# libsdl-org/libjxl

Hardware: AMD Instinct MI355X
Metric: megapixels/sec decode, 3840x2160 VarDCT d1.0 (higher is better)
Workload: dtype f32

## Files before the change

### libjxl_amd/csrc/hip/jxl_hip_entropy_lanes.h

```cpp
#ifndef JXL_HIP_ENTROPY_LANES_H_
#define JXL_HIP_ENTROPY_LANES_H_

#include "jxl_hip_kernels.h"
#include "jxl_hip_lanes_trip.inc"

namespace jxlhip {

struct EntropyLaneBatch {
  const EntropyParams* params;
  const uint32_t* wg_unit;
  const uint4* units;
  const uint32_t* list;
  uint32_t* queue;
  const uint8_t* wave_lanes;
  uint32_t prio;
  uint32_t extra_pass_min;
  uint32_t wait_shift;
  uint32_t refill_mask;
  const uint8_t* wave_log_ls;
  uint32_t debug;
  unsigned long long* started;
  unsigned long long* prof;
};

struct LanesLds {
  uint32_t f2, alias, ctx, ctx2, cfg, poff, wave0, per_wave, total;
};
constexpr uint32_t kLanesF2Bytes = 128;
constexpr uint32_t kLanesNzRows = 96;
constexpr uint32_t kLanesRingWords = 16;
constexpr uint32_t kLanesBlockRing = 8;
constexpr int kLanesTrips = 4;
constexpr uint32_t kLanesRefillEvery = 4;
constexpr uint32_t kLanesPerLaneBytes = kLanesNzRows + (kLanesRingWords + 2) * 4 + kLanesBlockRing * 4;
constexpr uint32_t kLanesA6Clusters = 128, kLanesA6Slots = 8192, kLanesA6B = 128, kLanesA6A = kLanesA6B + kLanesA6Slots * 2,
                   kLanesA6Cfg = kLanesA6A + kLanesA6Slots * 4, kLanesA6End = kLanesA6Cfg + kLanesA6Clusters * 2;
static_assert(kLanesA6A == 16512 && kLanesA6Cfg == 49280, "jxl_hip_lanes_trip.inc LT_EREAD_6 has these as immediates");
__host__ __device__ inline LanesLds LanesLdsLayout(uint32_t num_hist, uint32_t nctx, uint32_t num_clusters, uint32_t log_alpha,
                                                   uint32_t waves, uint32_t lanes, bool alias_lds = true, bool prefix = false, bool a6 = false) {
  LanesLds l;
  l.f2 = 0;
  l.alias = kLanesF2Bytes;
  l.ctx = a6 ? kLanesA6End : l.alias + (alias_lds ? (num_clusters << log_alpha) * 8 : 0);
  l.ctx2 = l.ctx + ((num_hist * nctx + 16 + 15) & ~15u);
  l.cfg = l.ctx2 + 64 * 2;
  l.poff = l.cfg + (prefix ? 256 * 2 : 0);
  l.wave0 = l.poff + (prefix ? 256 * 4 : 0);
  l.per_wave = kLanesPerLaneBytes * lanes;
  l.total = l.wave0 + waves * l.per_wave;
  return l;
}

typedef uint8_t __attribute__((address_space(3))) LdsU8;
typedef uint16_t __attribute__((address_space(3))) LdsU16;
typedef uint32_t __attribute__((address_space(3))) LdsU32;
typedef uint32_t LanesU32x2 __attribute__((ext_vector_type(2)));
typedef LanesU32x2 __attribute__((address_space(3))) LdsU32x2;

__device__ __forceinline__ void LaneStore64(const void* base, uint32_t off, uint32_t lo, uint32_t hi) {
  const LanesU32x2 v = {lo, hi};
  asm volatile("global_store_dwordx2 %0, %1, %2" : : "v"(off), "v"(v), "s"(base));
}
__device__ __forceinline__ void LaneStore32(const void* base, uint32_t off, uint32_t v) {
  asm volatile("global_store_dword %0, %1, %2" : : "v"(off), "v"(v), "s"(base));
}
__device__ __forceinline__ void LaneStore16(const void* base, uint32_t off, uint32_t v) {
  asm volatile("global_store_short %0, %1, %2" : : "v"(off), "v"(v), "s"(base));
}
__device__ __forceinline__ void LaneDmaDword(uint32_t lds_row, const void* base, uint32_t off) {
  uint32_t keep;
  asm volatile(
      "s_mov_b32 %0, m0\n\ts_mov_b32 m0, %2\n\ts_nop 0\n\tglobal_load_lds_dword %1, %3\n\ts_mov_b32 m0, %0"
      : "=&s"(keep)
      : "v"(off), "s"(lds_row), "s"(base)
      : "memory");
}
__device__ __forceinline__ void LaneDmaWait() { asm volatile("s_waitcnt vmcnt(0)" : : : "memory"); }
typedef uint32_t LanesU32x4 __attribute__((ext_vector_type(4)));
__device__ __forceinline__ void LaneLoad128(LanesU32x4& d, unsigned long long mask, const void* base, uint32_t off) {
  asm volatile("s_mov_b64 s[96:97], exec\n\ts_and_b64 exec, exec, %3\n\tglobal_load_dwordx4 %0, %1, %2\n\ts_mov_b64 exec, s[96:97]"
               : "+v"(d)
               : "v"(off), "s"(base), "s"(mask)
               : "memory", "s96", "s97", "scc");
}
__device__ __forceinline__ void LaneLoadWait(LanesU32x4& a, LanesU32x4& b) {
  asm volatile("s_waitcnt vmcnt(0)" : "+v"(a), "+v"(b) : : "memory");
}

__device__ __forceinline__ uint32_t LaneHybrid(uint32_t tok, uint32_t cfg, uint32_t w0, uint32_t w1, uint32_t w2, uint32_t boff,
                                               uint32_t& nb) {
  const uint32_t se = cfg & 15, msb = (cfg >> 4) & 15, lsb = (cfg >> 8) & 15;
  nb = (se - (msb + lsb) + ((tok - (1u << se)) >> (msb + lsb))) & 31u;
  const uint32_t low = tok & ((1u << lsb) - 1), top = tok >> lsb;
  const bool up = boff >= 32;
  const uint32_t xb = __builtin_amdgcn_alignbit(up ? w2 : w1, up ? w1 : w0, boff & 31) & ((1u << nb) - 1);
  return (((((1u << msb) | (top & ((1u << msb) - 1))) << nb) | xb) << lsb) | low;
}

template <typename CoefT, int WPG, bool AIDS, bool GALIAS = false, bool PREFIX = false, bool ASMT = false, bool A6 = false>
__global__ __launch_bounds__(64 * WPG) void k_entropy_lanes(EntropyLaneBatch B_) {
  static_assert(!ASMT || (!GALIAS && !PREFIX && sizeof(CoefT) == 2), "the assembly trip: LDS alias tables, int16 coefficients");
  static_assert(!A6 || (!GALIAS && !PREFIX), "the six-byte form is an LDS form of the rANS tables");
  EntropyLaneBatch B = B_;
  if (!AIDS) {
    B.prof = nullptr;
    B.debug = 0;
  }
  extern __shared__ __align__(16) uint8_t lds_raw[];
  if (B_.prio) __builtin_amdgcn_s_setprio(3);
  const uint32_t tid = threadIdx.x, lane = tid & 63;
  if (B_.started && tid == 0) __hip_atomic_fetch_add(B_.started, 1ull, __ATOMIC_RELAXED, __HIP_MEMORY_SCOPE_SYSTEM);
  const uint32_t wave = __builtin_amdgcn_readfirstlane(tid >> 6);
  typedef const uint32_t __attribute__((address_space(4)))* CU32;
  const uint32_t wid = blockIdx.x * WPG + wave;
  const uint32_t unit = ((CU32)(uintptr_t)B.wg_unit)[wid];
  const uint32_t wl = B.wave_log_ls[wid];
  const uint32_t lane_off = __builtin_amdgcn_readfirstlane(wl & 63), region = __builtin_amdgcn_readfirstlane((wl & 0x80) ? 0u : wave);
  const CU32 ud = (CU32)(uintptr_t)(B.units + unit);
  const uint32_t wg_desc = ud[0], list_begin = ud[1], list_count = ud[2], pass = ud[3];
  const uint32_t wg_sel = wg_desc >> 16;
  EntropyParams P;
  LoadParams(P, B.params + (wg_desc & 0xFFFF));
  PassDev T;
  LoadParams(T, P.passes + pass);
  const uint32_t log_alpha = T.log_alpha, log_entry = 12 - log_alpha, nclusters = T.num_clusters;
  const uint32_t entry_mask = (1u << log_entry) - 1, cl_shift = (A6 ? 1 : 3) + log_alpha;
  const uint32_t num_bctx = P.num_bctx, nctx = P.nctx, num_hist = P.num_hist;
  const LanesLds L = LanesLdsLayout(1, nctx, nclusters, log_alpha, 0, 0, !GALIAS && !PREFIX, PREFIX, A6);
  const uint2* const galias = T.alias_packed;
  const uint32_t* const ptable = T.prefix_table;
  LdsU8* const lds = (LdsU8*)lds_raw;
  auto alias_entry = [&](uint32_t cluster, uint32_t slot) -> LanesU32x2 {
    if constexpr (A6) {
      const uint32_t i = ((cluster << log_alpha) + slot) & (kLanesA6Slots - 1);
      const uint32_t b = ((LdsU16*)(lds + kLanesA6B))[i], a = ((LdsU32*)(lds + kLanesA6A))[i];
      const uint32_t cfg = ((LdsU16*)(lds + kLanesA6Cfg))[cluster & (kLanesA6Clusters - 1)];
      const uint32_t cutoff = (b >> 12) << (8 - log_alpha) | a >> (24 + log_alpha);
      return LanesU32x2{(b & 0xFFFu) | cfg << 12 | cutoff << 24, a & ((1u << (24 + log_alpha)) - 1)};
    } else {
      return *(LdsU32x2*)((LdsU8*)lds + kLanesF2Bytes + (cluster << cl_shift) + slot * 8);
    }
  };
  LdsU8* const l_ctx = lds + L.ctx;
  LdsU16* const l_nnz2 = (LdsU16*)(lds + L.ctx2);
  LdsU16* const l_cfg = (LdsU16*)(lds + L.cfg);
  LdsU32* const l_poff = (LdsU32*)(lds + L.poff);
  const uint32_t wave_base = L.wave0 + region * (kLanesPerLaneBytes * 64);
  const uint32_t col = lane_off + lane;
  LdsU8* const l_nz = lds + wave_base + col;
  const uint32_t ring_row0 = wave_base + kLanesNzRows * 64;
  const uint32_t bring_row0 = ring_row0 + (kLanesRingWords + 2) * 256;
  LdsU32* const ring = (LdsU32*)(lds + ring_row0) + col;
  LdsU32* const bring = (LdsU32*)(lds + bring_row0) + col;
  const uint32_t lds_abs = uint32_t(uintptr_t(lds)) + lane_off * 4;

  {
    const uint32_t n_ctx = nctx + 16;
// ... 109 lines not shown
      bool act = mode == kRun && !low;
      if constexpr (ASMT) {
        const unsigned long long actm = __ballot(act);
        if (actm) {
          unsigned long long th = 0;
          const uint32_t k_before = k;
          const uint32_t n_total = uint32_t(__popcll(actm)) + uint32_t(__popcll(__ballot(mode == kWait || mode == kFlush)));
          const uint32_t cont_min = __builtin_amdgcn_readfirstlane(((n_total << B.wait_shift) / (1u + (1u << B.wait_shift))) + 1u);
          uint32_t groups = 0;
          if (AIDS) {
            if (B.prof) th = __builtin_readcyclecounter();
            if constexpr (A6) {
              JXL_LANES_TRIP_LOOP6_COUNTED(groups, state, bitpos, k, nzeros, ctxe, addr_a, nnz_b, dst, acc_lo, acc_hi, log2c, cbase, covm2, ring_addr,
                                           ring_end, size, actm, cont_min, log_entry, entry_mask, cl_mul, nnz2_addr, shift, coef_base, log_alpha);
            } else {
              JXL_LANES_TRIP_LOOP_COUNTED(groups, state, bitpos, k, nzeros, ctxe, addr_a, nnz_b, dst, acc_lo, acc_hi, log2c, cbase, covm2, ring_addr,
                                          ring_end, size, actm, cont_min, log_entry, entry_mask, cl_mul, nnz2_addr, shift, coef_base, log_alpha);
            }
            if (B.prof) t_wait += __builtin_readcyclecounter() - th;
            n_trips += groups * kLanesTrips;
            n_calls++;
          } else {
            if constexpr (A6) {
              JXL_LANES_TRIP_LOOP6(groups, state, bitpos, k, nzeros, ctxe, addr_a, nnz_b, dst, acc_lo, acc_hi, log2c, cbase, covm2, ring_addr, ring_end,
                                   size, actm, cont_min, log_entry, entry_mask, cl_mul, nnz2_addr, shift, coef_base, log_alpha);
            } else {
              JXL_LANES_TRIP_LOOP(groups, state, bitpos, k, nzeros, ctxe, addr_a, nnz_b, dst, acc_lo, acc_hi, log2c, cbase, covm2, ring_addr, ring_end,
                                  size, actm, cont_min, log_entry, entry_mask, cl_mul, nnz2_addr, shift, coef_base, log_alpha);
            }
          }
          mode = (act && (nzeros == 0 || k >= size)) ? uint32_t(kFlush) : mode;
          if (AIDS && B.prof) n_lane_trips += act ? k - k_before : 0u;
          if (AIDS && (B.debug & 2)) ntok += act ? k - k_before : 0u;
        }
      } else
      if (__ballot(act)) {
        unsigned long long th = 0;
        if (B.prof) th = __builtin_readcyclecounter();
        if (AIDS) n_trips += kLanesTrips;
        uint32_t pw0 = 0, pw1 = 0, pw2 = 0, pe_zero = 0, pe_nonzero = 0, pnnz_c = 0;
        uint32_t ppo = 0, pcfg = 0, proot = 0;
        LanesU32x2 pe = {0, 0};
        auto request = [&]() {
          LdsU32* const rp = ring + ((bitpos >> 5) & (kLanesRingWords - 1)) * 64;
          if (PREFIX) {
            ppo = l_poff[ctxe & 255];
            pcfg = l_cfg[ctxe & 255];
          } else if (GALIAS) {
            if (act) {
              const uint2 ge = galias[(ctxe << log_alpha) + ((state & 0xFFFu) >> log_entry)];
              pe = LanesU32x2{ge.x, ge.y};
            }
          } else {
            pe = alias_entry(ctxe, (state & 0xFFFu) >> log_entry);
          }
          pw0 = rp[0];
          pw1 = rp[64];
          pw2 = rp[128];
          __builtin_amdgcn_sched_barrier(0);
          const uint32_t b = (k + 1) >> log2c;
          const uint32_t f2 = min(min(b - 1, 7 + (b >> 1)), 15 + (b >> 2)) << 1;
          pe_zero = l_ctx[(GALIAS || PREFIX) ? ((addr_a + f2) & 0x1FFF) : (addr_a + f2)];
          pe_nonzero = l_ctx[(GALIAS || PREFIX) ? ((cbase + 1 + nnz_b + f2) & 0x1FFF) : (cbase + 1 + nnz_b + f2)];
          pnnz_c = l_nnz2[((nzeros - 2 + covm1) >> log2c) & 63];
          if (PREFIX) {
            const uint32_t win = __builtin_amdgcn_alignbit(pw1, pw0, bitpos);
            proot = 0;
            if (act) proot = ptable[(ppo & 0xFFFFFFu) + (win & ((1u << (ppo >> 24)) - 1))];
          }
        };
        request();
#pragma unroll
        for (int rep = 0; rep < kLanesTrips; rep++) {
          if (AIDS && B.prof) n_lane_trips += act ? 1u : 0u;
          uint32_t w0, w1, w2, e_zero, e_nonzero, nnz_c;
          const uint32_t kn = k + 1;
          const uint32_t addr_b = cbase + 1 + nnz_b;
          uint32_t tok, cfg, adv, nstate = state;
          w0 = pw0, w1 = pw1, w2 = pw2, e_zero = pe_zero, e_nonzero = pe_nonzero, nnz_c = pnnz_c;
          if (PREFIX) {
            uint32_t e = proot;
            if (act && (e & 0x80u)) {
              const uint32_t win = __builtin_amdgcn_alignbit(w1, w0, bitpos);
              e = ptable[(ppo & 0xFFFFFFu) + (e >> 8) + ((win >> (ppo >> 24)) & ((1u << (e & 0x7Fu)) - 1))];
            }
            tok = e >> 8;
            adv = e & 0xFFu;
            cfg = pcfg;
          } else {
            const LanesU32x2 e = pe;
            const uint32_t res = state & 0xFFFu, slot = res >> log_entry, pos = res & entry_mask;
            const bool gt = pos >= (e.x >> 24);
            const uint32_t x = gt ? e.y : e.x;
            tok = gt ? (e.y >> 24) : slot;
            const uint32_t hi = state >> 12;
            nstate = (x & 0xFFFu) * hi + hi + (gt ? ((e.y >> 12) & 0xFFFu) : 0u) + pos;
            const bool need = nstate < (1u << 16);
            const uint32_t win = __builtin_amdgcn_alignbit(w1, w0, bitpos);
            nstate = need ? ((nstate << 16) | (win & 0xFFFFu)) : nstate;
            adv = need ? 16u : 0u;
            cfg = e.x >> 12;
          }
          const bool take = act && tok >= (1u << (cfg & 15));
          if (__ballot(take)) {
            uint32_t nbits;
            const uint32_t big = LaneHybrid(tok, cfg, w0, w1, w2, (bitpos & 31) + adv, nbits);
            tok = take ? big : tok;
            adv += take ? nbits : 0u;
          }
          const bool nz = tok != 0;
          const uint32_t n_nzeros = nzeros - (nz ? 1u : 0u);
          const bool done = n_nzeros == 0 || kn >= size;
          const bool full = act && (kn & (kPerChunk - 1)) == 0;
          const uint32_t acc_lo0 = acc_lo, acc_hi0 = acc_hi, dst0 = dst;
          state = act ? nstate : state;
          bitpos += act ? adv : 0u;
          k = act ? kn : k;
          nzeros = act ? n_nzeros : nzeros;
          ctxe = act ? (nz ? e_nonzero : e_zero) : ctxe;
          addr_a = (act && nz) ? addr_b - 1 : addr_a;
          nnz_b = (act && nz) ? nnz_c : nnz_b;
          if (rep + 1 < kLanesTrips) request();
          const uint32_t sgn = uint32_t(-int32_t(tok & 1));
          const int32_t coeff = int32_t(((tok >> 1) ^ sgn) << shift);
          uint32_t n_lo, n_hi;
          if (sizeof(CoefT) == 2) {
            n_lo = __builtin_amdgcn_alignbit(acc_hi0, acc_lo0, 16);
            n_hi = (acc_hi0 >> 16) | (uint32_t(coeff) << 16);
          } else {
            n_lo = acc_hi0;
            n_hi = uint32_t(coeff);
          }
          if ((B.debug & 1) == 0 && full) LaneStore64(coef_base, dst0, n_lo, n_hi);
          if (AIDS && (B.debug & 2)) ntok += act ? 1u : 0u;
          acc_lo = act ? n_lo : acc_lo0;
          acc_hi = act ? n_hi : acc_hi0;
          dst = dst0 + (full ? 8u : 0u);
          mode = (act && done) ? uint32_t(kFlush) : mode;
          act = act && !done;
        }
        if (B.prof) t_wait += __builtin_readcyclecounter() - th;
      }
    }
    {
      unsigned long long t2 = 0;
      if (B.prof) t2 = __builtin_readcyclecounter();
      const bool fl = mode == kFlush;
      const bool next_block = ci == 2 && started;
      const bool ran_out = fl && nzeros != 0;
      const bool rare = !started || (next_block && bi + 1 >= b1) || ran_out;
      const bool go = (mode == kWait || fl) && !rare && (ring_end - (bitpos >> 5)) >= 3 && (!next_block || bi + 1 < bring_end);
      const uint32_t n_go = uint32_t(__popcll(__ballot(fl || go))), n_run = uint32_t(__popcll(__ballot(mode == kRun)));
      if (n_go && (n_go << B.wait_shift) >= n_run) {
        if (ASMT) {
          if (fl) {
            const uint32_t part = (k - covm1 - 1) & 3;
            if (!(B.debug & 1)) {
              if (part >= 2) LaneStore32(coef_base, dst, acc_lo);
              if (part & 1) LaneStore16(coef_base, dst + (part & 2) * 2, part == 3 ? acc_hi : acc_lo);
            }
            if (!(B.debug & 4)) LaneStore32(kend_base, kidx * 4, k);
          }
        } else
        if (fl) {
          const uint32_t part = k & (kPerChunk - 1);
          const uint64_t v = ((uint64_t(acc_hi) << 32) | acc_lo) >> (((kPerChunk - part) & (kPerChunk - 1)) * (64 / kPerChunk));
          if (!(B.debug & 1) && part) LaneStore64(coef_base, dst, uint32_t(v), uint32_t(v >> 32));
          if (!(B.debug & 4)) LaneStore32(kend_base, kidx * 4, k);
        }
        err |= ran_out ? kErrNzeros : 0u;
        bi = ran_out ? b1 : bi;
        ci = ran_out ? 2u : ci;
        mode = fl ? uint32_t(kWait) : mode;
        if constexpr (ASMT) {
          if (go) {
            const bool nb = ci == 2;
            const uint32_t n_ci = nb ? 0u : ci + 1, n_bi = bi + (nb ? 1u : 0u);
            if (nb) {
              info = bring[(n_bi & (kLanesBlockRing - 1)) * 64];
              coef_offset = next_offset;
            }
            const uint32_t n_log2c = ((info >> 6) & 7) + ((info >> 9) & 7);
            if (nb) next_offset += 64u << n_log2c;
            const uint32_t c = n_ci == 0 ? 1u : (n_ci == 1 ? 0u : 2u);
            if ((info >> (24 + c)) & 1u) {
              if (!(B.debug & 4)) LaneStore32(kend_base, (n_bi * 3 + c) * 4, 0);
              bi = n_bi;
              ci = n_ci;
            } else {
            const uint32_t n_lbx = (info & 31) >> ((info >> (27 + c)) & 1u), n_lby = (info >> 5) & 1;
            const uint32_t log2cx = (info >> 6) & 7;
            const uint32_t bctx = (info >> (12 + 4 * c)) & 15;
            LdsU8* line = l_nz + (c * 32) * 64;
            const uint32_t top = line[n_lbx * 64], left = line[(n_lbx ? n_lbx - 1 : 0) * 64];
            const uint32_t l0 = n_lbx ? left : 32u, tt = n_lby ? top : l0, ll = n_lbx ? left : tt;
            const uint32_t pred = (tt + ll + 1) >> 1;
            uint32_t nzb = pred >= 64 ? 64 : pred;
            nzb = nzb < 8 ? nzb : 4 + nzb / 2;
            const uint32_t cluster = l_ctx[(nzb * num_bctx + bctx) & 0x1FFF];
            const uint32_t slotw = (bitpos >> 5) & (kLanesRingWords - 1);
            const uint32_t w0 = ring[slotw * 64], w1 = ring[slotw * 64 + 64], w2 = ring[slotw * 64 + 128];
            const uint32_t res = state & 0xFFFu, slot = res >> log_entry, pos = res & entry_mask;
            const LanesU32x2 e = alias_entry(cluster, slot);
            const bool gt = pos >= (e.x >> 24);
            const uint32_t x = gt ? e.y : e.x;
            uint32_t tok = gt ? (e.y >> 24) : slot;
            const uint32_t hi = state >> 12;
            uint32_t nstate = (x & 0xFFFu) * hi + hi + (gt ? ((e.y >> 12) & 0xFFFu) : 0u) + pos;
            const bool need = nstate < (1u << 16);
            const uint32_t win = __builtin_amdgcn_alignbit(w1, w0, bitpos);
            state = need ? ((nstate << 16) | (win & 0xFFFFu)) : nstate;
            uint32_t adv = need ? 16u : 0u;
            const uint32_t cfg = e.x >> 12;
            const bool take = tok >= (1u << (cfg & 15));
            if (__ballot(take)) {
              uint32_t nbits;
              const uint32_t big = LaneHybrid(tok, cfg, w0, w1, w2, (bitpos & 31) + adv, nbits);
              tok = take ? big : tok;
              adv += take ? nbits : 0u;
            }
            bitpos += adv;
            const uint32_t covered = 1u << n_log2c;
            log2c = n_log2c;
            size = covered * 64;
            kidx = n_bi * 3 + c;
            const bool bad = tok > size - covered;
            const uint8_t nzv = uint8_t((tok + covered - 1) >> n_log2c);
            if (!bad) {
              line[n_lbx * 64] = nzv;
              if (__ballot(log2cx != 0)) {
                const uint32_t cx = 1u << log2cx;
                for (uint32_t i = 1; i < cx; i++) line[(n_lbx + i) * 64] = nzv;
              }
            }
            if (tok == 0 && !(B.debug & 4)) LaneStore32(kend_base, kidx * 4, 0);
            covm1 = covered - 1;
            covm2 = covered - 3;
            const uint32_t n_cbase = num_bctx * 37 + 458 * bctx;
            const uint32_t prev = tok > size / 16 ? 0 : 1;
            const uint32_t n_addr_a = n_cbase + l_nnz2[((tok + covm1) >> n_log2c) & 63];
            nnz_b = l_nnz2[((tok - 1 + covm1) >> n_log2c) & 63];
            ctxe = l_ctx[(n_addr_a + prev) & 0x1FFF];
            cbase = n_cbase + L.ctx;
            addr_a = n_addr_a + L.ctx;
            dst = uint32_t(((g * 3 + c) * 65536 + coef_offset + covered) * sizeof(CoefT));
            nzeros = tok;
            k = covered;
            mode = (tok != 0 && !bad) ? uint32_t(kRun) : mode;
            err |= bad ? kErrNzeros : 0u;
            bi = bad ? b1 : n_bi;
            ci = bad ? 2u : n_ci;
            }
          }
        } else {
        const bool nb = ci == 2;
        const uint32_t n_ci = nb ? 0u : ci + 1, n_bi = bi + (nb ? 1u : 0u);
        const uint32_t rec = bring[(n_bi & (kLanesBlockRing - 1)) * 64];
        const uint32_t n_info = nb ? rec : info;
        const uint32_t n_log2c = ((n_info >> 6) & 7) + ((n_info >> 9) & 7);
        const uint32_t n_coef_offset = nb ? next_offset : coef_offset;
        const uint32_t c = n_ci == 0 ? 1u : (n_ci == 1 ? 0u : 2u);
        const bool absent = ((n_info >> (24 + c)) & 1u) != 0;
        const bool go_all = go;
        const bool go = go_all && !absent;
        const uint32_t n_lbx = (n_info & 31) >> ((n_info >> (27 + c)) & 1u), n_lby = (n_info >> 5) & 1;
        const uint32_t log2cx = (n_info >> 6) & 7;
        const uint32_t bctx = (n_info >> (12 + 4 * c)) & 15;
        LdsU8* line = l_nz + (c * 32) * 64;
        const uint32_t top = line[n_lbx * 64], left = line[(n_lbx ? n_lbx - 1 : 0) * 64];
        const uint32_t l0 = n_lbx ? left : 32u, tt = n_lby ? top : l0, ll = n_lbx ? left : tt;
        const uint32_t pred = (tt + ll + 1) >> 1;
        uint32_t nzb = pred >= 64 ? 64 : pred;
        nzb = nzb < 8 ? nzb : 4 + nzb / 2;
        const uint32_t cluster = l_ctx[(nzb * num_bctx + bctx) & 0x1FFF];
        const uint32_t slotw = (bitpos >> 5) & (kLanesRingWords - 1);
        const uint32_t w0 = ring[slotw * 64], w1 = ring[slotw * 64 + 64], w2 = ring[slotw * 64 + 128];
        uint32_t tok, cfg, adv, nstate = state;
        if (PREFIX) {
          const uint32_t po = l_poff[cluster];
          const uint32_t win = __builtin_amdgcn_alignbit(w1, w0, bitpos);
          uint32_t e = 0;
          if (go) e = PrefixLookup(ptable + (po & 0xFFFFFFu), po >> 24, win);
          tok = e >> 8;
          adv = e & 0xFFu;
          cfg = l_cfg[cluster];
        } else {
          const uint32_t res = state & 0xFFFu, slot = res >> log_entry, pos = res & entry_mask;
          LanesU32x2 e = {0, 0};
          if (GALIAS) {
            if (go) {
              const uint2 ge = galias[(cluster << log_alpha) + slot];
              e = LanesU32x2{ge.x, ge.y};
            }
          } else {
            e = alias_entry(cluster, slot);
          }
          const bool gt = pos >= (e.x >> 24);
          const uint32_t x = gt ? e.y : e.x;
          tok = gt ? (e.y >> 24) : slot;
          const uint32_t hi = state >> 12;
          nstate = (x & 0xFFFu) * hi + hi + (gt ? ((e.y >> 12) & 0xFFFu) : 0u) + pos;
          const bool need = nstate < (1u << 16);
          const uint32_t win = __builtin_amdgcn_alignbit(w1, w0, bitpos);
          nstate = need ? ((nstate << 16) | (win & 0xFFFFu)) : nstate;
          adv = need ? 16u : 0u;
          cfg = e.x >> 12;
        }
        const bool take = go && tok >= (1u << (cfg & 15));
        if (__ballot(take)) {
          uint32_t nbits;
          const uint32_t big = LaneHybrid(tok, cfg, w0, w1, w2, (bitpos & 31) + adv, nbits);
          tok = take ? big : tok;
          adv += take ? nbits : 0u;
        }
        const uint32_t covered = 1u << n_log2c, n_size = covered * 64;
        const uint32_t n_kidx = n_bi * 3 + c;
        const bool bad = tok > n_size - covered;
        const uint8_t nzv = uint8_t((tok + covered - 1) >> n_log2c);
        if (go && !bad) {
          line[n_lbx * 64] = nzv;
          if (__ballot(log2cx != 0)) {
            const uint32_t cx = 1u << log2cx;
            for (uint32_t i = 1; i < cx; i++) line[(n_lbx + i) * 64] = nzv;
          }
        }
        if (((go && tok == 0) || (go_all && absent)) && !(B.debug & 4)) LaneStore32(kend_base, n_kidx * 4, 0);
        const uint32_t n_covm1 = covered - 1;
        const uint32_t n_cbase = num_bctx * 37 + 458 * bctx;
        const uint32_t prev = tok > n_size / 16 ? 0 : 1;
        const uint32_t n_addr_a = n_cbase + l_nnz2[((tok + n_covm1) >> n_log2c) & 63];
        const uint32_t n_nnz_b = l_nnz2[((tok - 1 + n_covm1) >> n_log2c) & 63];
        const uint32_t n_ctxe = l_ctx[(n_addr_a + prev) & 0x1FFF];
        state = go ? nstate : state;
        bitpos += go ? adv : 0u;
        info = go_all ? n_info : info;
        coef_offset = go_all ? n_coef_offset : coef_offset;
        next_offset += (go_all && nb) ? (64u << n_log2c) : 0u;
        log2c = go ? n_log2c : log2c;
        size = go ? n_size : size;
        kidx = go ? n_kidx : kidx;
        nzeros = go ? tok : nzeros;
        k = go ? covered : k;
        covm1 = go ? n_covm1 : covm1;
        if (ASMT) {
          covm2 = go ? n_covm1 - 2 : covm2;
          cbase = go ? n_cbase + L.ctx : cbase;
          dst = go ? uint32_t(((g * 3 + c) * 65536 + n_coef_offset + covered) * sizeof(CoefT)) : dst;
          addr_a = go ? n_addr_a + L.ctx : addr_a;
        } else {
        cbase = go ? n_cbase : cbase;
        dst = go ? uint32_t(((g * 3 + c) * 65536 + n_coef_offset + (covered & ~(kPerChunk - 1))) * sizeof(CoefT)) : dst;
        acc_lo = go ? 0u : acc_lo;
        acc_hi = go ? 0u : acc_hi;
        addr_a = go ? n_addr_a : addr_a;
        }
        nnz_b = go ? n_nnz_b : nnz_b;
        ctxe = go ? n_ctxe : ctxe;
        mode = (go && tok != 0 && !bad) ? uint32_t(kRun) : mode;
        err |= (go && bad) ? kErrNzeros : 0u;
        bi = go_all ? ((go && bad) ? b1 : n_bi) : bi;
        ci = go_all ? ((go && bad) ? 2u : n_ci) : ci;
        }
        if (B.prof) {
          t_trans += __builtin_readcyclecounter() - t2;
          n_service++;
          t_dma += n_go;
        }
      }
    }
    if ((++round & B.refill_mask) != 0) continue;
    {
      unsigned long long t0 = 0;
      if (B.prof) t0 = __builtin_readcyclecounter();
      if (!__ballot(mode != kDone)) break;
      if constexpr (ASMT) {
        if (__ballot(stg_n | btg_n)) LaneLoadWait(stg, btg);
        if (__ballot(stg_n != 0)) {
          if (stg_n) {
            const bool zeros = stg_n == 8;
            const uint32_t s0 = zeros ? 0u : stg.x, s1 = zeros ? 0u : stg.y, s2 = zeros ? 0u : stg.z, s3 = zeros ? 0u : stg.w;
            LdsU32* const r4 = ring + (ring_end & (kLanesRingWords - 1)) * 64;
            r4[0] = s0;
            r4[64] = s1;
            r4[128] = s2;
            r4[192] = s3;
            if ((ring_end & (kLanesRingWords - 1)) == 0) {
              ring[16 * 64] = s0;
              ring[17 * 64] = s1;
            }
            ring_end += 4;
            stg_n = 0;
          }
        }
        if (__ballot(btg_n != 0)) {
          if (btg_n) {
            LdsU32* const r4 = bring + (bring_end & (kLanesBlockRing - 1) & ~3u) * 64;
            r4[0] = btg.x;
            r4[64] = btg.y;
            r4[128] = btg.z;
            r4[192] = btg.w;
            bring_end = (bring_end & ~3u) + 4;
            btg_n = 0;
          }
        }
      } else {
      LaneDmaWait();
      ring_end += pend_s;
      bring_end += pend_b;
      pend_s = pend_b = 0;
      }
      {
        const bool next_block = ci == 2 && started;
        const bool rare = mode == kWait && (ring_end - (bitpos >> 5)) >= 3 && (!started || (next_block && bi + 1 >= b1));
        if (__ballot(rare)) {
          if (rare) {
            if (!started) {
              started = true;
              uint32_t hb = 0;
              while ((1u << hb) < num_hist) hb++;
              const uint32_t w0 = ring[0], w1 = ring[64];
              const uint64_t win = ((uint64_t(w1) << 32) | w0) >> bitpos;
              const uint32_t sel = hb ? uint32_t(win) & ((1u << hb) - 1) : 0;
              if (sel != wg_sel) err = kErrSelector;
              state = PREFIX ? 0x13u << 16 : uint32_t(win >> hb);
              bitpos += hb + (PREFIX ? 0 : 32);
            } else {
              if (state != (0x13u << 16)) err |= kErrFinalState;
              if (bitpos > sec_size * 8) err |= kErrOverread;
              P.sec_end_bits[sec0 + g] = bitpos;
              if (P.num_passes > 1) atomicOr(P.errors + g, err);
              else P.errors[g] = (B.debug & 2) ? ntok : err;
              ntok = 0;
              g = take_section();
              if (g == 0xFFFFFFFFu) mode = kDone;
              else open_section();
            }
          }
          __builtin_amdgcn_s_waitcnt(0);
        }
      }
      if constexpr (ASMT) {
        const uint32_t used = ring_end - (bitpos >> 5);
        const bool want_s = mode != kDone && kLanesRingWords - used >= 4;
        const bool want_b = mode != kDone && bring_end < b1 && (bi + 1 + kLanesBlockRing - bring_end) >= 4;
        const unsigned long long ms = __ballot(want_s && ring_end < nwords), mb = __ballot(want_b);
        if (ms) LaneLoad128(stg, ms, P.sections, sec_off + ring_end * 4);
        if (mb) LaneLoad128(btg, mb, P.block_recs, (bring_end & ~3u) * 4);
        stg_n = want_s ? (ring_end < nwords ? 4u : 8u) : 0u;
        btg_n = want_b ? 4u : 0u;
      } else {
        const uint32_t used = ring_end - (bitpos >> 5);
        const uint32_t groups_s = mode == kDone ? 0u : (kLanesRingWords - used) >> 2;
        const uint32_t first_g = (ring_end >> 2) & 3;
        const uint32_t next_b = bi + 1;
        const uint32_t bfirst = (bring_end >> 2) & 1;
        uint32_t groups_b = 0;
        if (mode != kDone && bring_end < b1) groups_b = (next_b + kLanesBlockRing - bring_end) >> 2;
        if (__ballot(groups_s != 0)) {
#pragma unroll
          for (uint32_t gi = 0; gi < 4; gi++) {
            const uint32_t d = (gi - first_g) & 3;
            const bool in = d < groups_s;
            const uint32_t w = ring_end + d * 4;
            const bool beyond = w >= nwords;
            dma_group4(in && !beyond, lds_abs + ring_row0 + gi * 1024, P.sections, sec_off + w * 4);
            if (gi == 0) {
              if (in && !beyond) {
                LaneDmaDword(lds_abs + ring_row0 + 16 * 256, P.sections, sec_off + w * 4);
                LaneDmaDword(lds_abs + ring_row0 + 17 * 256, P.sections, sec_off + w * 4 + 4);
              }
            }
            if (__ballot(in && beyond)) {
              if (in && beyond) {
                for (uint32_t j = 0; j < 4; j++) ring[(gi * 4 + j) * 64] = 0;
                if (gi == 0) ring[16 * 64] = ring[17 * 64] = 0;
              }
            }
          }
          pend_s = groups_s * 4;
        }
        if (__ballot(groups_b != 0)) {
#pragma unroll
          for (uint32_t gi = 0; gi < 2; gi++) {
            const uint32_t d = (gi - bfirst) & 1;
            const bool in = d < groups_b;
            dma_group4(in, lds_abs + bring_row0 + gi * 1024, P.block_recs, ((bring_end & ~3u) + d * 4) * 4);
          }
          pend_b = groups_b * 4 - (groups_b ? (bring_end & 3) : 0);
        }
      }
      if (B.prof) t_service += __builtin_readcyclecounter() - t0;
    }
  }
  if (B.prof && lane == 0) {
    unsigned long long* o = B.prof + size_t(blockIdx.x * WPG + wave) * 8;
    o[0] = __builtin_readcyclecounter() - t_begin;
    o[1] = t_service;
    o[2] = n_service;
    o[3] = n_trips;
    o[5] = t_wait;
    o[6] = t_dma;
    o[7] = t_trans;
    if (B.debug & 32) o[6] = n_calls;
    if (B.debug & 16) {
      uint32_t hw, xcc;
      asm volatile("s_getreg_b32 %0, hwreg(HW_REG_HW_ID)" : "=s"(hw));
      asm volatile("s_getreg_b32 %0, hwreg(HW_REG_XCC_ID)" : "=s"(xcc));
      o[6] = (unsigned long long)hw | ((unsigned long long)xcc << 32);
    }
  }
  if (B.prof) {
    unsigned long long total = n_lane_trips;
    for (int off = 32; off; off >>= 1) total += __shfl_down(total, off);
    if (lane == 0) B.prof[size_t(blockIdx.x * WPG + wave) * 8 + 4] = total;
  }
// ... 5 lines not shown
```

Before: 91340.

## Replace ASMT flush/transition service path with hand-written inline assembly

```diff
diff --git a/libjxl_amd/csrc/hip/jxl_hip_entropy_lanes.h b/libjxl_amd/csrc/hip/jxl_hip_entropy_lanes.h
--- a/libjxl_amd/csrc/hip/jxl_hip_entropy_lanes.h
+++ b/libjxl_amd/csrc/hip/jxl_hip_entropy_lanes.h
@@ -3,6 +3,7 @@
 
 #include "jxl_hip_kernels.h"
 #include "jxl_hip_lanes_trip.inc"
+#include "jxl_hip_lanes_pass.inc"
 
 namespace jxlhip {
 
@@ -418,6 +419,20 @@
       const bool go = (mode == kWait || fl) && !rare && (ring_end - (bitpos >> 5)) >= 3 && (!next_block || bi + 1 < bring_end);
       const uint32_t n_go = uint32_t(__popcll(__ballot(fl || go))), n_run = uint32_t(__popcll(__ballot(mode == kRun)));
       if (n_go && (n_go << B.wait_shift) >= n_run) {
+        if (ASMT && !(B.debug & 5)) {
+          const unsigned long long flm = __ballot(fl), gom = __ballot(go);
+          const uint32_t bring_addr = uint32_t(uintptr_t(bring)), lnz_addr = uint32_t(uintptr_t(l_nz));
+          const uint32_t nbc37 = num_bctx * 37, ctx_addr = L.ctx;
+          if constexpr (A6) {
+            JXL_LANES_PASS6(state, bitpos, k, nzeros, ctxe, addr_a, nnz_b, dst, cbase, covm2, log2c, size, kidx, info, coef_offset,
+                            next_offset, bi, ci, mode, err, acc_lo, acc_hi, g, b1, ring_addr, bring_addr, lnz_addr, flm, gom,
+                            log_entry, entry_mask, cl_mul, nnz2_addr, num_bctx, nbc37, ctx_addr, coef_base, kend_base, log_alpha);
+          } else {
+            JXL_LANES_PASS(state, bitpos, k, nzeros, ctxe, addr_a, nnz_b, dst, cbase, covm2, log2c, size, kidx, info, coef_offset,
+                           next_offset, bi, ci, mode, err, acc_lo, acc_hi, g, b1, ring_addr, bring_addr, lnz_addr, flm, gom,
+                           log_entry, entry_mask, cl_mul, nnz2_addr, num_bctx, nbc37, ctx_addr, coef_base, kend_base, log_alpha);
+          }
+        } else {
         if (ASMT) {
           if (fl) {
             const uint32_t part = (k - covm1 - 1) & 3;
@@ -438,87 +453,7 @@
         bi = ran_out ? b1 : bi;
         ci = ran_out ? 2u : ci;
         mode = fl ? uint32_t(kWait) : mode;
-        if constexpr (ASMT) {
-          if (go) {
-            const bool nb = ci == 2;
-            const uint32_t n_ci = nb ? 0u : ci + 1, n_bi = bi + (nb ? 1u : 0u);
-            if (nb) {
-              info = bring[(n_bi & (kLanesBlockRing - 1)) * 64];
-              coef_offset = next_offset;
-            }
-            const uint32_t n_log2c = ((info >> 6) & 7) + ((info >> 9) & 7);
-            if (nb) next_offset += 64u << n_log2c;
-            const uint32_t c = n_ci == 0 ? 1u : (n_ci == 1 ? 0u : 2u);
-            if ((info >> (24 + c)) & 1u) {
-              if (!(B.debug & 4)) LaneStore32(kend_base, (n_bi * 3 + c) * 4, 0);
-              bi = n_bi;
-              ci = n_ci;
-            } else {
-            const uint32_t n_lbx = (info & 31) >> ((info >> (27 + c)) & 1u), n_lby = (info >> 5) & 1;
-            const uint32_t log2cx = (info >> 6) & 7;
-            const uint32_t bctx = (info >> (12 + 4 * c)) & 15;
-            LdsU8* line = l_nz + (c * 32) * 64;
-            const uint32_t top = line[n_lbx * 64], left = line[(n_lbx ? n_lbx - 1 : 0) * 64];
-            const uint32_t l0 = n_lbx ? left : 32u, tt = n_lby ? top : l0, ll = n_lbx ? left : tt;
-            const uint32_t pred = (tt + ll + 1) >> 1;
-            uint32_t nzb = pred >= 64 ? 64 : pred;
-            nzb = nzb < 8 ? nzb : 4 + nzb / 2;
-            const uint32_t cluster = l_ctx[(nzb * num_bctx + bctx) & 0x1FFF];
-            const uint32_t slotw = (bitpos >> 5) & (kLanesRingWords - 1);
-            const uint32_t w0 = ring[slotw * 64], w1 = ring[slotw * 64 + 64], w2 = ring[slotw * 64 + 128];
-            const uint32_t res = state & 0xFFFu, slot = res >> log_entry, pos = res & entry_mask;
-            const LanesU32x2 e = alias_entry(cluster, slot);
-            const bool gt = pos >= (e.x >> 24);
-            const uint32_t x = gt ? e.y : e.x;
-            uint32_t tok = gt ? (e.y >> 24) : slot;
-            const uint32_t hi = state >> 12;
-            uint32_t nstate = (x & 0xFFFu) * hi + hi + (gt ? ((e.y >> 12) & 0xFFFu) : 0u) + pos;
-            const bool need = nstate < (1u << 16);
-            const uint32_t win = __builtin_amdgcn_alignbit(w1, w0, bitpos);
-            state = need ? ((nstate << 16) | (win & 0xFFFFu)) : nstate;
-            uint32_t adv = need ? 16u : 0u;
-            const uint32_t cfg = e.x >> 12;
-            const bool take = tok >= (1u << (cfg & 15));
-            if (__ballot(take)) {
-              uint32_t nbits;
-              const uint32_t big = LaneHybrid(tok, cfg, w0, w1, w2, (bitpos & 31) + adv, nbits);
-              tok = take ? big : tok;
-              adv += take ? nbits : 0u;
-            }
-            bitpos += adv;
-            const uint32_t covered = 1u << n_log2c;
-            log2c = n_log2c;
-            size = covered * 64;
-            kidx = n_bi * 3 + c;
-            const bool bad = tok > size - covered;
-            const uint8_t nzv = uint8_t((tok + covered - 1) >> n_log2c);
-            if (!bad) {
-              line[n_lbx * 64] = nzv;
-              if (__ballot(log2cx != 0)) {
-                const uint32_t cx = 1u << log2cx;
-                for (uint32_t i = 1; i < cx; i++) line[(n_lbx + i) * 64] = nzv;
-              }
-            }
-            if (tok == 0 && !(B.debug & 4)) LaneStore32(kend_base, kidx * 4, 0);
-            covm1 = covered - 1;
-            covm2 = covered - 3;
-            const uint32_t n_cbase = num_bctx * 37 + 458 * bctx;
-            const uint32_t prev = tok > size / 16 ? 0 : 1;
-            const uint32_t n_addr_a = n_cbase + l_nnz2[((tok + covm1) >> n_log2c) & 63];
-            nnz_b = l_nnz2[((tok - 1 + covm1) >> n_log2c) & 63];
-            ctxe = l_ctx[(n_addr_a + prev) & 0x1FFF];
-            cbase = n_cbase + L.ctx;
-            addr_a = n_addr_a + L.ctx;
-            dst = uint32_t(((g * 3 + c) * 65536 + coef_offset + covered) * sizeof(CoefT));
-            nzeros = tok;
-            k = covered;
-            mode = (tok != 0 && !bad) ? uint32_t(kRun) : mode;
-            err |= bad ? kErrNzeros : 0u;
-            bi = bad ? b1 : n_bi;
-            ci = bad ? 2u : n_ci;
-            }
-          }
-        } else {
+        {
         const bool nb = ci == 2;
         const uint32_t n_ci = nb ? 0u : ci + 1, n_bi = bi + (nb ? 1u : 0u);
         const uint32_t rec = bring[(n_bi & (kLanesBlockRing - 1)) * 64];
@@ -627,6 +562,7 @@
         bi = go_all ? ((go && bad) ? b1 : n_bi) : bi;
         ci = go_all ? ((go && bad) ? 2u : n_ci) : ci;
         }
+        }
         if (B.prof) {
           t_trans += __builtin_readcyclecounter() - t2;
           n_service++;
diff --git a/libjxl_amd/csrc/hip/jxl_hip_lanes_pass.inc b/libjxl_amd/csrc/hip/jxl_hip_lanes_pass.inc
--- /dev/null
+++ b/libjxl_amd/csrc/hip/jxl_hip_lanes_pass.inc
@@ -0,0 +1,261 @@
+#ifndef JXL_HIP_LANES_PASS_INC_
+#define JXL_HIP_LANES_PASS_INC_
+
+#include "jxl_hip_lanes_trip.inc"
+
+#define LP_REC "v104"
+#define LP_C "v105"
+#define LP_L2X "v106"
+#define LP_BCTX "v108"
+#define LP_CBR "v109"
+#define LP_TOPA "v110"
+#define LP_X "v111"
+#define LP_TOP "v130"
+#define LP_LEFT "v131"
+
+#define LP_EREAD_8                                                                                                   \
+  "v_lshlrev_b32 " LT_T4 ", 3, " LT_SL "\n\t"                                                                        \
+  "v_mad_u32_u24 " LT_T4 ", " LT_T0 ", %[clm], " LT_T4 "\n\t"                                                        \
+  "ds_read_b64 " LT_E ", " LT_T4 " offset:128\n\t"
+#define LP_EREAD_6                                                                                                   \
+  "v_lshlrev_b32 " LT_T4 ", 1, " LT_SL "\n\t"                                                                        \
+  "v_mad_u32_u24 " LT_T4 ", " LT_T0 ", %[clm], " LT_T4 "\n\t"                                                        \
+  "v_lshlrev_b32 " LT_TB ", 1, " LT_T0 "\n\t"                                                                        \
+  "v_lshlrev_b32 " LT_TA ", 1, " LT_T4 "\n\t"                                                                        \
+  "ds_read_u16 " LT_E0 ", " LT_T4 " offset:128\n\t"                                                                  \
+  "ds_read_b32 " LT_E1 ", " LT_TA " offset:16512\n\t"                                                                \
+  "ds_read_u16 " LT_CF ", " LT_TB " offset:49280\n\t"
+
+#define JXL_LANES_PASS_(V, p_st, p_bp, p_k, p_nzl, p_ctxe, p_aa, p_nb, p_dst, p_cb, p_covm2, p_log2c, p_size, p_kidx, p_info, p_coff,  \
+                        p_noff, p_bi, p_ci, p_mode, p_err, p_alo, p_ahi, p_g, p_b1, p_ring, p_bring, p_lnz, p_fl, p_go, p_le, p_em,   \
+                        p_clm, p_nnz2, p_nbc, p_nbc37, p_ctx, p_coef, p_kend, p_la)                                                 \
+  asm volatile(                                                                                                                \
+      "s_mov_b64 s[96:97], exec\n\t"                                                                                           \
+                \
+                          \
+      "s_mov_b64 exec, %[fl]\n\t"                                                                                              \
+      "s_cbranch_execz .Llp_go_%=\n\t"                                                                                         \
+      "v_sub_u32 " LT_T0 ", %[k], %[covm2]\n\t"                                                                                \
+      "v_lshlrev_b32 " LT_T2 ", 2, %[kidx]\n\t"                                                                                \
+      "v_add_u32 " LT_T0 ", 1, " LT_T0 "\n\t"                                                                                  \
+      "global_store_dword " LT_T2 ", %[k], %[kend]\n\t"                                                                        \
+      "v_and_b32 " LT_T0 ", 3, " LT_T0 "\n\t"                                                                       \
+      "v_add_u32 " LT_T3 ", 4, %[dst]\n\t"                                                                                     \
+      "v_cmp_lt_u32 vcc, 1, " LT_T0 "\n\t"                                    \
+      "v_and_b32 " LT_T1 ", 1, " LT_T0 "\n\t"                                                                                  \
+      "v_cmp_ne_u32_e64 s[98:99], 0, " LT_T1 "\n\t"                                                    \
+      "v_cndmask_b32 " LT_T4 ", %[alo], %[ahi], vcc\n\t"                                                                       \
+      "v_cndmask_b32 " LT_T3 ", %[dst], " LT_T3 ", vcc\n\t"                                                                    \
+      "s_and_saveexec_b64 s[100:101], vcc\n\t"                                                                                 \
+      "global_store_dword %[dst], %[alo], %[coef]\n\t"                                                                         \
+      "s_and_b64 exec, s[100:101], s[98:99]\n\t"                                                                               \
+      "global_store_short " LT_T3 ", " LT_T4 ", %[coef]\n\t"                                                                   \
+      "s_mov_b64 exec, %[fl]\n\t"                                                                                              \
+      "v_cmp_ne_u32 vcc, 0, %[nzl]\n\t"                                              \
+      "v_mov_b32 %[mode], 0\n\t"                                                                                 \
+      "v_or_b32 " LT_T5 ", 1, %[err]\n\t"                                                                     \
+      "v_cndmask_b32 %[err], %[err], " LT_T5 ", vcc\n\t"                                                                       \
+      "v_cndmask_b32 %[bi], %[bi], %[b1], vcc\n\t"                                                                             \
+      "v_cndmask_b32_e64 %[ci], %[ci], 2, vcc\n"                                                                               \
+      ".Llp_go_%=:\n\t"                                                                                                        \
+                               \
+      "s_mov_b64 exec, %[go]\n\t"                                                                                              \
+      "s_cbranch_execz .Llp_end_%=\n\t"                                                                                        \
+      "v_cmp_eq_u32_e64 s[100:101], 2, %[ci]\n\t"                                                   \
+      "v_add_u32 " LT_T0 ", 1, %[ci]\n\t"                                                                                      \
+      "v_bfe_u32 " LT_RA ", %[bp], 5, 4\n\t"                                                                                   \
+      "v_lshl_add_u32 " LT_RA ", " LT_RA ", 8, %[ring]\n\t"                                                                    \
+      "v_addc_co_u32_e64 %[bi], s[98:99], 0, %[bi], s[100:101]\n\t"                                                            \
+      "v_cndmask_b32_e64 %[ci], " LT_T0 ", 0, s[100:101]\n\t"                                                                  \
+      "v_and_b32 " LP_X ", 7, %[bi]\n\t"                                                                                       \
+      "v_lshl_add_u32 " LP_X ", " LP_X ", 8, %[bring]\n\t"                                                                     \
+      "ds_read_b32 " LP_REC ", " LP_X "\n\t"                                                                                   \
+      "ds_read2_b32 " LT_W ", " LT_RA " offset1:64\n\t"                                                \
+      "ds_read_b32 " LT_W2 ", " LT_RA " offset:512\n\t"                                                                        \
+      "v_xor_b32 " LP_C ", 1, %[ci]\n\t"                                                                                       \
+      "v_and_b32 " LT_RS ", 0xfff, %[st]\n\t"                                                                                  \
+      "v_min_u32 " LP_C ", 2, " LP_C "\n\t"                                                                      \
+      "v_lshrrev_b32 " LT_SL ", %[le], " LT_RS "\n\t"                                            \
+      "v_mad_u32_u24 %[kidx], %[bi], 3, " LP_C "\n\t"                                                                          \
+      "v_lshlrev_b32 " LP_X ", 11, " LP_C "\n\t"                                       \
+      "v_add_u32 " LP_X ", %[lnz], " LP_X "\n\t"                                                                               \
+      "v_add_u32 " LT_T5 ", 27, " LP_C "\n\t"                                                                                  \
+      "v_lshl_add_u32 " LT_T6 ", " LP_C ", 2, 12\n\t"                                                                          \
+      "v_add_u32 " LT_T7 ", 24, " LP_C "\n\t"                                                                                  \
+      LT_WAITCNT("2")                                                                                         \
+      "v_cndmask_b32_e64 %[info], %[info], " LP_REC ", s[100:101]\n\t"                                                         \
+      "v_cndmask_b32_e64 %[coff], %[coff], %[noff], s[100:101]\n\t"       \
+            \
+                                               \
+      "v_bfe_u32 " LT_T4 ", %[info], " LT_T7 ", 1\n\t"                                                                         \
+      "v_bfe_u32 " LP_L2X ", %[info], 6, 3\n\t"                                                                                \
+      "v_bfe_u32 " LT_T8 ", %[info], 9, 3\n\t"                                                                                 \
+      "v_cmp_ne_u32_e64 s[98:99], 0, " LT_T4 "\n\t"                                                       \
+      "v_add_u32 %[log2c], " LP_L2X ", " LT_T8 "\n\t"                                                                          \
+      "v_and_b32 " LT_T4 ", 31, %[info]\n\t"                                                                                   \
+      "v_lshlrev_b32_e64 %[size], %[log2c], 64\n\t"                                                                            \
+      "v_bfe_u32 " LT_T5 ", %[info], " LT_T5 ", 1\n\t"                                                                         \
+      "v_cndmask_b32_e64 " LT_T8 ", 0, %[size], s[100:101]\n\t"                                                                \
+      "v_lshrrev_b32 " LT_T4 ", " LT_T5 ", " LT_T4 "\n\t"                           \
+      "v_add_u32 %[noff], %[noff], " LT_T8 "\n\t"                                                                              \
+      "s_cmp_lg_u64 s[98:99], 0\n\t"                                                                                           \
+      "s_cbranch_scc0 .Llp_present_%=\n\t"                                                                                     \
+                                   \
+      "s_mov_b64 exec, s[98:99]\n\t"                                                                                           \
+      "v_mov_b32 " LT_T8 ", 0\n\t"                                                                                             \
+      "v_lshlrev_b32 " LT_T5 ", 2, %[kidx]\n\t"                                                                                \
+      "global_store_dword " LT_T5 ", " LT_T8 ", %[kend]\n\t"                                                                   \
+      "s_andn2_b64 exec, %[go], s[98:99]\n\t"                                                                                  \
+      "s_cbranch_execz .Llp_wait_%=\n"                                                                                         \
+      ".Llp_present_%=:\n\t"                                                                                                   \
+                            \
+      "v_lshl_add_u32 " LP_TOPA ", " LT_T4 ", 6, " LP_X "\n\t"                                                                 \
+      "v_cmp_ne_u32 vcc, 0, " LT_T4 "\n\t"                                                          \
+      "v_subrev_u32 " LP_X ", 64, " LP_TOPA "\n\t"                                                                             \
+      "v_bfe_u32 " LP_BCTX ", %[info], " LT_T6 ", 4\n\t"                                                                       \
+      "v_and_b32 " LT_T5 ", 32, %[info]\n\t"                                                                                   \
+      "v_cndmask_b32 " LP_X ", " LP_TOPA ", " LP_X ", vcc\n\t"                                                                 \
+      "ds_read_u8 " LP_TOP ", " LP_TOPA "\n\t"                                                                                 \
+      "ds_read_u8 " LP_LEFT ", " LP_X "\n\t"                                                                                   \
+      "v_cmp_ne_u32_e64 s[98:99], 0, " LT_T5 "\n\t"                                                    \
+      "v_mul_u32_u24 " LP_CBR ", 0x1ca, " LP_BCTX "\n\t"                                             \
+      "v_and_b32 " LT_T1 ", %[em], %[st]\n\t"                                          \
+      "v_add_u32 " LP_CBR ", %[nbc37], " LP_CBR "\n\t"                                                                         \
+      "v_lshrrev_b32 " LT_T3 ", 12, %[st]\n\t"                                                                                 \
+      "v_add_u32 %[cb], %[ctx], " LP_CBR "\n\t"                                                                                \
+      LT_WAITCNT("0")                                                                                                          \
+      "v_cndmask_b32 " LT_T0 ", 32, " LP_LEFT ", vcc\n\t"                                                                      \
+      "v_cndmask_b32_e64 " LT_T0 ", " LT_T0 ", " LP_TOP ", s[98:99]\n\t"                                                       \
+      "v_cndmask_b32 " LT_T2 ", " LT_T0 ", " LP_LEFT ", vcc\n\t"                                                               \
+      "v_add3_u32 " LT_T0 ", " LT_T0 ", " LT_T2 ", 1\n\t"                                                                      \
+      "v_lshrrev_b32 " LT_T0 ", 1, " LT_T0 "\n\t"                                                                              \
+      "v_min_u32 " LT_T0 ", 64, " LT_T0 "\n\t"                                                                                 \
+      "v_lshrrev_b32 " LT_T2 ", 1, " LT_T0 "\n\t"                                                                              \
+      "v_cmp_gt_u32 vcc, 8, " LT_T0 "\n\t"                                                                                     \
+      "v_add_u32 " LT_T2 ", 4, " LT_T2 "\n\t"                                                                                  \
+      "s_nop 0\n\t"                                                                                                            \
+      "v_cndmask_b32 " LT_T0 ", " LT_T2 ", " LT_T0 ", vcc\n\t"                                                                 \
+      "v_mad_u32_u24 " LT_T0 ", " LT_T0 ", %[nbc], " LP_BCTX "\n\t"                                                            \
+      "v_and_b32 " LT_T0 ", 0x1fff, " LT_T0 "\n\t"                                                                             \
+      "v_add_u32 " LT_T0 ", %[ctx], " LT_T0 "\n\t"                                                                             \
+      "ds_read_u8 " LT_T0 ", " LT_T0 "\n\t"                                                                  \
+      LT_WAITCNT("0")                                                                                                          \
+                                                                                  \
+      LP_EREAD_##V                                                                                                             \
+      LT_WAITCNT("0")                                                                                                          \
+      LT_HEAD_##V                                                                                                              \
+      "v_bfe_u32 " LT_T5 ", " LT_E1 ", 12, 12\n\t"                                                              \
+      "v_cmp_lt_u32 vcc, " LT_T1 ", " LT_T0 "\n\t"                                   \
+      LT_SPLIT_##V                                                                                                             \
+      "s_nop 0\n\t"                                                                                                            \
+      "v_cndmask_b32 " LT_T4 ", " LT_E1 ", " LT_E0 ", vcc\n\t"                                                                 \
+      "v_cndmask_b32 " LT_T2 ", " LT_T2 ", " LT_SL ", vcc\n\t"                                                 \
+      "v_cndmask_b32_e64 " LT_T5 ", " LT_T5 ", 0, vcc\n\t"                                                                     \
+      "v_and_b32 " LT_T4 ", 0xfff, " LT_T4 "\n\t"                                                               \
+      "v_lshrrev_b32 " LT_T8 ", " LT_T7 ", " LT_T2 "\n\t"                                        \
+      "v_mad_u32_u24 " LT_T4 ", " LT_T4 ", " LT_T3 ", " LT_T3 "\n\t"                                                           \
+      "v_cmp_ne_u32_e64 s[98:99], 0, " LT_T8 "\n\t"                                               \
+      "v_add3_u32 " LT_T4 ", " LT_T4 ", " LT_T5 ", " LT_T1 "\n\t"                       \
+      "v_alignbit_b32 " LT_T5 ", " LT_W1 ", " LT_W0 ", %[bp]\n\t"                                                              \
+      "v_cmp_gt_u32 vcc, %[c64k], " LT_T4 "\n\t"                                               \
+      "v_perm_b32 " LT_T5 ", " LT_T4 ", " LT_T5 ", %[perm]\n\t"                                                                \
+      "v_lshlrev_b32_e64 " LT_T0 ", %[log2c], 1\n\t"                                                             \
+      "v_cndmask_b32 %[st], " LT_T4 ", " LT_T5 ", vcc\n\t"                                                 \
+      "v_cndmask_b32_e64 " LT_T6 ", 0, 16, vcc\n\t"                                                                            \
+      "s_cmp_lg_u64 s[98:99], 0\n\t"                                                                                           \
+      "s_cbranch_scc0 .Llp_skip_%=\n\t"                                                                                        \
+                                                 \
+      "s_and_saveexec_b64 s[100:101], s[98:99]\n\t"                                                                            \
+      LT_MSB_##V                                                                                                               \
+      LT_LSB_##V                                                                                                               \
+      "v_alignbit_b32 " LT_TC ", " LT_W1 ", " LT_W0 ", %[bp]\n\t"                                                              \
+      "v_alignbit_b32 " LT_TD ", " LT_W2 ", " LT_W1 ", %[bp]\n\t"                                                              \
+      "v_lshl_add_u32 " LT_TB ", -1, " LT_T7 ", " LT_T2 "\n\t"                                                                 \
+      "v_add_u32 " LT_TA ", " LT_T8 ", " LT_T9 "\n\t"                                                                          \
+      "v_lshrrev_b64 " LT_TCD ", " LT_T6 ", " LT_TCD "\n\t"                                                                    \
+      "v_lshrrev_b32 " LT_TB ", " LT_TA ", " LT_TB "\n\t"                                                                      \
+      "v_sub_u32 " LT_TA ", " LT_T7 ", " LT_TA "\n\t"                                                                          \
+      "v_add_u32 " LT_TB ", " LT_TA ", " LT_TB "\n\t"                                                                          \
+      "v_bfe_u32 " LT_TA ", " LT_T2 ", " LT_T9 ", " LT_T8 "\n\t"                                                               \
+      "v_bfe_u32 " LT_TC ", " LT_TC ", 0, " LT_TB "\n\t"                                                                       \
+      "v_and_b32 " LT_TD ", 31, " LT_TB "\n\t"                                                                                 \
+      "v_lshl_or_b32 " LT_TA ", 1, " LT_T8 ", " LT_TA "\n\t"                                                                   \
+      "v_add_u32 " LT_T6 ", " LT_T6 ", " LT_TD "\n\t"                                                                          \
+      "v_lshl_or_b32 " LT_TA ", " LT_TA ", " LT_TB ", " LT_TC "\n\t"                                                           \
+      "v_bfe_u32 " LT_TC ", " LT_T2 ", 0, " LT_T9 "\n\t"                                                                       \
+      "v_lshl_or_b32 " LT_T2 ", " LT_TA ", " LT_T9 ", " LT_TC "\n\t"                                                           \
+      "s_mov_b64 exec, s[100:101]\n"                                                                                           \
+      ".Llp_skip_%=:\n\t"                                                                                                      \
+                                                        \
+      "v_sub_u32 " LT_T1 ", %[size], " LT_T0 "\n\t"                                                                            \
+      "v_add3_u32 " LT_T3 ", " LT_T2 ", " LT_T0 ", -1\n\t"                                           \
+      "v_cmp_le_u32_e64 s[98:99], " LT_T2 ", " LT_T1 "\n\t"                                              \
+      "v_add3_u32 " LT_T4 ", " LT_T2 ", " LT_T0 ", -2\n\t"                                                                     \
+      "v_bfe_u32 " LT_T5 ", " LT_T3 ", %[log2c], 6\n\t"                                                                        \
+      "v_bfe_u32 " LT_T4 ", " LT_T4 ", %[log2c], 6\n\t"                                                                        \
+      "v_lshl_add_u32 " LT_T5 ", " LT_T5 ", 1, %[nnz2]\n\t"                                                                    \
+      "v_lshl_add_u32 " LT_T4 ", " LT_T4 ", 1, %[nnz2]\n\t"                                                                    \
+      "ds_read_u16 " LT_T5 ", " LT_T5 "\n\t"                                             \
+      "ds_read_u16 %[nb], " LT_T4 "\n\t"                                                                   \
+      "v_add_u32 %[bp], %[bp], " LT_T6 "\n\t"                                                                                  \
+      "v_lshrrev_b32 " LT_T3 ", %[log2c], " LT_T3 "\n\t"                                                  \
+      "v_lshrrev_b32 " LT_T4 ", 4, %[size]\n\t"                                                                                \
+      "v_mad_u32_u24 " LT_T6 ", %[g], 3, " LP_C "\n\t"                                                                         \
+      "v_cmp_le_u32 vcc, " LT_T2 ", " LT_T4 "\n\t"                        \
+      "v_add_u32 %[covm2], -3, " LT_T0 "\n\t"                                                                                  \
+      "v_lshl_add_u32 " LT_T6 ", " LT_T6 ", 16, %[coff]\n\t"                                                                   \
+      "v_mov_b32 %[nzl], " LT_T2 "\n\t"                                                                                        \
+      "v_add_lshl_u32 %[dst], " LT_T6 ", " LT_T0 ", 1\n\t"                                    \
+      "v_mov_b32 %[k], " LT_T0 "\n\t"                                                                                          \
+      LT_WAITCNT("1")                                                                                                          \
+      "v_add_u32 %[aa], %[cb], " LT_T5 "\n\t"                                                                                  \
+      "v_addc_co_u32 " LT_T5 ", vcc, " LP_CBR ", " LT_T5 ", vcc\n\t"                                         \
+      "v_and_b32 " LT_T5 ", 0x1fff, " LT_T5 "\n\t"                                                                             \
+      "v_add_u32 " LT_T5 ", %[ctx], " LT_T5 "\n\t"                                                                             \
+      "ds_read_u8 %[ctxe], " LT_T5 "\n\t"                                          \
+                                                      \
+      "v_cmp_eq_u32 vcc, 0, " LT_T2 "\n\t"                                                                                     \
+      "v_mov_b32 " LT_T4 ", 0\n\t"                                                                                             \
+      "v_lshlrev_b32 " LT_T5 ", 2, %[kidx]\n\t"                                                                                \
+      "s_and_saveexec_b64 s[100:101], vcc\n\t"                                                                                 \
+      "global_store_dword " LT_T5 ", " LT_T4 ", %[kend]\n\t"                                                                   \
+      "s_andn2_b64 exec, s[100:101], vcc\n\t"                                                                                  \
+      "s_and_b64 vcc, exec, s[98:99]\n\t"                                           \
+      "s_andn2_b64 exec, s[100:101], s[98:99]\n\t"                               \
+      "v_or_b32 %[err], 1, %[err]\n\t"                                                                        \
+      "v_mov_b32 %[bi], %[b1]\n\t"                                                                                             \
+      "v_mov_b32 %[ci], 2\n\t"                                                                                                 \
+      "s_and_b64 exec, s[100:101], s[98:99]\n\t"                                       \
+      "v_cndmask_b32_e64 %[mode], %[mode], 1, vcc\n\t"                                                              \
+      "ds_write_b8 " LP_TOPA ", " LT_T3 "\n\t"                                                                                 \
+      "v_cmp_ne_u32 vcc, 0, " LP_L2X "\n\t"                              \
+      "v_lshlrev_b32_e64 " LT_T4 ", " LP_L2X ", 1\n\t"                                                                         \
+      "s_and_b64 exec, exec, vcc\n\t"                                                                                          \
+      "s_cbranch_execz .Llp_wait_%=\n"                                                                                         \
+      ".Llp_wide_%=:\n\t"                                                                                                      \
+      "v_add_u32 " LP_TOPA ", 64, " LP_TOPA "\n\t"                                                                             \
+      "v_subrev_u32 " LT_T4 ", 1, " LT_T4 "\n\t"                                                                               \
+      "ds_write_b8 " LP_TOPA ", " LT_T3 "\n\t"                                                                                 \
+      "v_cmp_lt_u32 vcc, 1, " LT_T4 "\n\t"                                                                                     \
+      "s_and_b64 exec, exec, vcc\n\t"                                                                                          \
+      "s_cbranch_execnz .Llp_wide_%=\n"                                                                                        \
+      ".Llp_wait_%=:\n\t"                                                                                                      \
+      "s_waitcnt lgkmcnt(0)\n"                                                                                                 \
+      ".Llp_end_%=:\n\t"                                                                                                       \
+      "s_mov_b64 exec, s[96:97]"                                                                                               \
+      : [st] "+v"(p_st), [bp] "+v"(p_bp), [k] "+v"(p_k), [nzl] "+v"(p_nzl), [ctxe] "+v"(p_ctxe), [aa] "+v"(p_aa), [nb] "+v"(p_nb), \
+        [dst] "+v"(p_dst), [cb] "+v"(p_cb), [covm2] "+v"(p_covm2), [log2c] "+v"(p_log2c), [size] "+v"(p_size),                   \
+        [kidx] "+v"(p_kidx), [info] "+v"(p_info), [coff] "+v"(p_coff), [noff] "+v"(p_noff), [bi] "+v"(p_bi), [ci] "+v"(p_ci),   \
+        [mode] "+v"(p_mode), [err] "+v"(p_err)                                                                                   \
+      : [alo] "v"(p_alo), [ahi] "v"(p_ahi), [g] "v"(p_g), [b1] "v"(p_b1), [ring] "v"(p_ring), [bring] "v"(p_bring),              \
+        [lnz] "v"(p_lnz), [fl] "s"(p_fl), [go] "s"(p_go), [le] "s"(p_le), [em] "s"(p_em), [clm] "s"(p_clm), [nnz2] "s"(p_nnz2), \
+        [nbc] "s"(p_nbc), [nbc37] "s"(p_nbc37), [ctx] "s"(p_ctx), [coef] "s"(p_coef), [kend] "s"(p_kend),                        \
+        [perm] "s"(0x05040100u), [c64k] "s"(0x10000u), [a6la] "s"(p_la), [a6s1] "s"(8u - (p_la)), [a6s2] "s"(24u + (p_la))       \
+      : "memory", "vcc", "scc", "s96", "s97", "s98", "s99", "s100", "s101", "v100", "v101", "v102", "v103",    \
+        "v104", "v105", "v106", "v107", "v108", "v109", "v110", "v111", "v112", "v113", "v114", "v115", "v116", "v117", "v118", \
+        "v119", "v120", "v121", "v122", "v123", "v124", "v125", "v126", "v127", "v128", "v129", "v130", "v131")
+
+#define JXL_LANES_PASS(...) JXL_LANES_PASS_(8, __VA_ARGS__)
+#define JXL_LANES_PASS6(...) JXL_LANES_PASS_(6, __VA_ARGS__)
+
+#endif
```

Measured after the change: 91560, median of 6. Within noise of the previous version (+0.2%).
